# zuds-survey/zuds-pipeline

Measured on AMD Instinct MI355X. Metric: Mpix/s resample->coadd->subtract, 3072x3072 frames, higher is better.
Workload: dtype f32; 1 GPU; configs[1]+[2]: 32x 3072x3072 TPV frames/GPU, mesh background + weight rescale + Lanczos-3 resample + WEIGHTED coadd (+ AND mask coadd, int16 masks); then 1 science frame/GPU: align ref, hotpants 3x3 regions x 10x10 stamps, r=10, ko=4, subtract; frames_per_gpu=32, size=3072, mask_dtype=int16, combine=WEIGHTED, subtract=True

## Files before the change

### zuds-pipeline_amd/csrc/background.hip

```cpp
#include <algorithm>

#include "zm_internal.h"

#define BK_BIG 1e30f
#define BK_NLEVELS 4096
#define BK_THREADS 256

__device__ inline double block_sum(double v, double* red) {
#pragma unroll
    for (int o = 32; o >= 1; o >>= 1) v += __shfl_xor(v, o);
    const int wave = threadIdx.x >> 6;
    __syncthreads();
    if ((threadIdx.x & 63) == 0) red[wave] = v;
    __syncthreads();
    return (red[0] + red[1]) + (red[2] + red[3]);
}

#define BK_PER (BK_NLEVELS / BK_THREADS)

struct mesh_lds {
    int histo[BK_NLEVELS];
    long long b1[BK_THREADS];
    long long b2[BK_THREADS];
    double red[4];
// ... 200 lines not shown
    }
    __syncthreads();
    if ((threadIdx.x & 63) == 0) {
        red[0][threadIdx.x >> 6] = a;
        red[1][threadIdx.x >> 6] = b;
        red[2][threadIdx.x >> 6] = c;
    }
    __syncthreads();
    a = b = c = 0.0;
#pragma unroll
    for (int w = 0; w < BKF_WAVES; ++w) { a += red[0][w]; b += red[1][w]; c += red[2][w]; }
}

#define BK_BATCH 64
struct bk_batch {
    const float* img[BK_BATCH];
    const float* wgt[BK_BATCH];
};

__device__ __forceinline__ void mesh_general(float (&v)[BKF_PX], const int area, meshf_lds* S,
                                             mesh_dump* __restrict__ D, const int dbg, const float khint,
                                             const int rot0) {
    const int tid = threadIdx.x;
    const float qnan = __builtin_nanf("");
    float kf = khint;
    if (!(khint == khint)) {
#pragma unroll
    for (int k = BKF_PX - 1; k >= 0; --k) kf = (v[k] == v[k]) ? v[k] : kf;
    {
        const unsigned long long has = __ballot(kf == kf);
        const int src = has ? __ffsll((long long)has) - 1 : 0;
        kf = __shfl(kf, src);
        __syncthreads();
        if ((tid & 63) == 0) S->red[tid >> 6] = (double)kf;
        __syncthreads();
        double kd = __builtin_nan("");
#pragma unroll
        for (int w8 = BKF_WAVES - 1; w8 >= 0; --w8) { const double c = S->red[w8]; kd = (c == c) ? c : kd; }
        kf = (float)kd;
    }
    }
    if (!(kf == kf)) {
        if (tid == 0) D->valid = 0;
        return;
    }
    const double K = (double)kf;
    for (int k = tid; k < BK_NLEVELS; k += BKF_THREADS) S->histo[k] = 0;
    double s0 = 0, s1 = 0, s2 = 0;
    {
        int cnt = 0;
#pragma unroll
        for (int k = 0; k < BKF_PX; ++k) {
            const float x = v[k];
            const bool in = (x == x);
            const double d = (double)(in ? x : kf) - K;
            cnt += in ? 1 : 0;
            s1 += d;
            s2 = fma(d, d, s2);
        }
        s0 = (double)cnt;
    }
    blockf_sum3_1b(s0, s1, s2, S->rot[rot0 % 3]);
    if (s0 < area * 0.5 || s0 < 1.0) {
        if (tid == 0) D->valid = 0;
        return;
    }
    double dm = s1 / s0;
    double var = s2 / s0 - dm * dm;
    double sig = var > 0 ? sqrt(var) : 0.0;
    const bool allsame = sig == 0.0;
    const double lc = K + dm - 2.0 * sig, hc = K + dm + 2.0 * sig;
    s0 = s1 = s2 = 0;
    {
        float lcf = (float)lc, hcf = (float)hc;
        if ((double)lcf < lc) lcf = nextafterf(lcf, INFINITY);
        if ((double)hcf > hc) hcf = nextafterf(hcf, -INFINITY);
        int cnt = 0;
#pragma unroll
        for (int k = 0; k < BKF_PX; ++k) {
            const float x = v[k];
            const bool in = (x >= lcf) && (x <= hcf);
            const double d = (double)(in ? x : kf) - K;
            cnt += in ? 1 : 0;
            s1 += d;
            s2 = fma(d, d, s2);
        }
        s0 = (double)cnt;
    }
    blockf_sum3_1b(s0, s1, s2, S->rot[(rot0 + 1) % 3]);
    if (s0 < 1.0) {
        if (tid == 0) D->valid = 0;
        return;
    }
    dm = s1 / s0;
    const double mean = K + dm;
    var = s2 / s0 - dm * dm;
    sig = var > 0 ? sqrt(var) : 0.0;
    const bk_quant q = make_quant(mean, sig, s0);
    if (dbg == 2) { if (sig == 12345.0) D->valid = 7; return; }
    if (allsame) {
        if (tid == 0) {
                        D->q = q;
            D->mean0 = (double)(float)mean;
            D->valid = 2;
        }
        return;
    }
    {
        const float qinv = 1.0f / q.qscale;
        const bool slow_div = (__float_as_uint(q.qscale) & 0x7fffffu) == 0x7fffffu;
        if (!slow_div) {
#pragma unroll
            for (int k = 0; k < BKF_PX; ++k) {
                const float x = v[k];
                const float q0 = x * qinv;
                const float qq = fmaf(fmaf(-q0, q.qscale, x), qinv, q0);
                const int b = (int)(qq + q.cste);
                if ((x == x) && b >= 0 && b < q.nlevels) atomicAdd(&S->histo[b], 1);
            }
        } else {
#pragma unroll
            for (int k = 0; k < BKF_PX; ++k) {
                const float x = v[k];
                const int b = (int)(x / q.qscale + q.cste);
                if ((x == x) && b >= 0 && b < q.nlevels) atomicAdd(&S->histo[b], 1);
            }
        }
    }
    __syncthreads();
    if (dbg == 3) { if (S->histo[tid] == -5) D->valid = 7; return; }
    {
        constexpr int NB = BK_NLEVELS / BKF_THREADS;
        static_assert(NB == 8 || NB == 4, "the histogram hand-over packs 8 or 4 bins per thread");
        const int4 lo = *reinterpret_cast<const int4*>(&S->histo[NB * tid]);
        if (NB == 8) {
            const int4 hi = *reinterpret_cast<const int4*>(&S->histo[NB * tid + 4]);
            int4 o;
            o.x = (int)((unsigned)lo.x | ((unsigned)lo.y << 16));
            o.y = (int)((unsigned)lo.z | ((unsigned)lo.w << 16));
            o.z = (int)((unsigned)hi.x | ((unsigned)hi.y << 16));
            o.w = (int)((unsigned)hi.z | ((unsigned)hi.w << 16));
            reinterpret_cast<int4*>(D->h)[tid] = o;
        } else {
            int2 o;
            o.x = (int)((unsigned)lo.x | ((unsigned)lo.y << 16));
            o.y = (int)((unsigned)lo.z | ((unsigned)lo.w << 16));
            reinterpret_cast<int2*>(D->h)[tid] = o;
        }
        if (tid == 0) { D->q = q; D->mean0 = (double)(float)mean; D->valid = 1; }
    }
}

#ifndef BKF_WPS
#define BKF_WPS 4
#endif
template <int SEL>
__global__ __launch_bounds__(BKF_THREADS, BKF_WPS) void k_mesh_stats_fast(const bk_batch B, int nx, int ny, int mesh,
                                                                 int nbx, int nby, float wthresh, int vec_ok,
                                                                 int dbg, mesh_dump* __restrict__ dump) {
    extern __shared__ char smem_raw[];
    meshf_lds* S = reinterpret_cast<meshf_lds*>(smem_raw);
    constexpr int NM = SEL == 2 ? 2 : 1;
    const int frame = blockIdx.z;
    const float* __restrict__ img = B.img[frame];
    const float* __restrict__ wgt = B.wgt[frame];
    const int mi = blockIdx.x, mj = blockIdx.y;
    const int x0 = mi * mesh, y0 = mj * mesh;
    const int w = min(mesh, nx - x0), h = min(mesh, ny - y0);
    const int area = w * h;
    const int tid = threadIdx.x;
    const float qnan = __builtin_nanf("");
    mesh_dump* D0 = dump + ((size_t)(frame * NM) * nby + mj) * nbx + mi;
    mesh_dump* D1 = D0 + (size_t)(NM - 1) * nby * nbx;

    float v[BKF_PX];
    float wmn = __builtin_inff(), wmx = -__builtin_inff();
    int wcnt = 0;
    const float pinf = __builtin_inff();
    const float thr = wgt ? wthresh : -pinf;
    float khint = qnan;
    if (SEL != 1) {
        const size_t i00 = (size_t)y0 * nx + x0;
        const float p0 = img[i00], w0 = wgt ? wgt[i00] : 1.f;
        khint = (w0 > thr && fabsf(p0) < BK_BIG) ? p0 : qnan;
    }
    const int c4 = (tid & 31) * 4, r32 = tid >> 5;
#pragma unroll
    for (int k = 0; k < BKF_PX / 4; ++k) {
        const int row = BKF_ROWS * k + r32;
        float pv[4] = {qnan, qnan, qnan, qnan};
        float pw[4] = {-pinf, -pinf, -pinf, -pinf};
        if (row < h && c4 < w) {
            const size_t idx = (size_t)(y0 + row) * nx + x0 + c4;
            if (vec_ok && c4 + 3 < w) {
                if (SEL != 1) {
                    float4 a = *reinterpret_cast<const float4*>(img + idx);
                    pv[0] = a.x; pv[1] = a.y; pv[2] = a.z; pv[3] = a.w;
                }
                if (wgt) {
                    float4 b = *reinterpret_cast<const float4*>(wgt + idx);
                    pw[0] = b.x; pw[1] = b.y; pw[2] = b.z; pw[3] = b.w;
                } else {
                    pw[0] = pw[1] = pw[2] = pw[3] = 1.f;
                }
            } else {
#pragma unroll
                for (int j = 0; j < 4; ++j)
                    if (c4 + j < w) {
                        if (SEL != 1) pv[j] = img[idx + j];
                        pw[j] = wgt ? wgt[idx + j] : 1.f;
                    }
            }
        }
#pragma unroll
        for (int j = 0; j < 4; ++j) {
            const float x = pw[j];
            const bool good = x > thr;
            if (SEL != 0) {
                const bool in = good && (x > -BK_BIG);
                wmn = fminf(wmn, in ? x : pinf);
                wmx = fmaxf(wmx, in ? x : -pinf);
                wcnt += in ? 1 : 0;
                if (SEL == 1) v[4 * k + j] = in ? x : qnan;
            }
            if (SEL != 1) {
                const float val = pv[j];
                v[4 * k + j] = (good && (fabsf(val) < BK_BIG)) ? val : qnan;
            }
        }
    }
    if (dbg == 1) {
        float a = 0.f;
#pragma unroll
        for (int k = 0; k < BKF_PX; ++k) a += v[k];
        if (a == 12345.f) dump[0].valid = 7;
        return;
    }
    bool flat = false;
    if (SEL != 0) {
#pragma unroll
        for (int o = 32; o >= 1; o >>= 1) {
            wmn = fminf(wmn, __shfl_xor(wmn, o));
            wmx = fmaxf(wmx, __shfl_xor(wmx, o));
            wcnt += __shfl_xor(wcnt, o);
        }
        if ((tid & 63) == 0) { S->red3[0][tid >> 6] = wmn; S->red3[1][tid >> 6] = wmx; S->red3[2][tid >> 6] = wcnt; }
        __syncthreads();
        double bmn = S->red3[0][0], bmx = S->red3[1][0], bc = 0.0;
#pragma unroll
        for (int w8 = 0; w8 < BKF_WAVES; ++w8) {
            bmn = fmin(bmn, S->red3[0][w8]);
            bmx = fmax(bmx, S->red3[1][w8]);
            bc += S->red3[2][w8];
        }
        const float inv = 1.0f / (float)bmn;
        flat = bc >= 1.0 && bc >= area * 0.5 && bmn == bmx && inv > -BK_BIG && inv == inv;
        if (flat && tid == 0) {
            D1->q = make_quant((double)inv, 0.0, bc);
            D1->mean0 = (double)inv;
            D1->valid = 2;
        }
    }
    if (SEL != 1) mesh_general(v, area, S, D0, dbg, khint, 0);
    if (SEL == 0 || flat) return;
    if (SEL == 2) {
        __syncthreads();
#pragma unroll
        for (int k = 0; k < BKF_PX / 4; ++k) {
            const int row = BKF_ROWS * k + r32;
#pragma unroll
            for (int j = 0; j < 4; ++j) {
                float x = qnan;
                if (row < h && c4 + j < w) x = wgt[(size_t)(y0 + row) * nx + x0 + c4 + j];
                v[4 * k + j] = (x > wthresh && x > -BK_BIG) ? x : qnan;
            }
        }
    }
#pragma unroll
    for (int k = 0; k < BKF_PX; ++k) {
        const float x = v[k];
        const float val = 1.0f / x;
        const bool ok = (x == x) && (fabsf(val) < BK_BIG);
        v[k] = ok ? val : qnan;
    }
    __syncthreads();
    mesh_general(v, area, S, D1, dbg, qnan, 2);
}

__global__ __launch_bounds__(64) void k_mesh_guess(const mesh_dump* __restrict__ dump, int n, int nmode,
                                                   int nslot, float* __restrict__ raw) {
    __shared__ __attribute__((aligned(16))) unsigned short P0[BK_NLEVELS];
    __shared__ long long B1[BK_THREADS];
    __shared__ long long B2[BK_THREADS];
    const int m = blockIdx.x, z = blockIdx.y, lane = threadIdx.x;
    const int frame = z / nmode, mode = z - frame * nmode;
    const mesh_dump* D = dump + (size_t)z * n + m;
    float* ob = raw + (size_t)frame * 4 * nslot + (size_t)mode * 2 * n + m;
    float* os = ob + n;
    if (!D->valid) {
        if (lane == 0) { *ob = -BK_BIG; *os = -BK_BIG; }
        return;
    }
    if (D->valid == 2) {
        if (lane == 0) { *ob = D->q.qzero; *os = 0.f; }
        return;
    }
    const int4* src = reinterpret_cast<const int4*>(D->h);
    int4 piece[BK_NLEVELS / 8 / 64];
#pragma unroll
    for (int k = 0; k < BK_NLEVELS / 8 / 64; ++k) piece[k] = src[k * 64 + lane];
    unsigned run0 = 0;
    long long run1 = 0, run2 = 0;
#pragma unroll
    for (int k = 0; k < BK_NLEVELS / 8 / 64; ++k) {
        const unsigned wv[4] = {(unsigned)piece[k].x, (unsigned)piece[k].y, (unsigned)piece[k].z, (unsigned)piece[k].w};
        unsigned c[8];
#pragma unroll
        for (int j = 0; j < 4; ++j) { c[2 * j] = wv[j] & 0xffffu; c[2 * j + 1] = wv[j] >> 16; }
        unsigned s0 = 0, s1 = 0, s2 = 0;
#pragma unroll
        for (int j = 0; j < 8; ++j) { s0 += c[j]; s1 += c[j] * (unsigned)j; s2 += c[j] * (unsigned)(j * j); }
        const long long base = (long long)(512 * k + 8 * lane);
        const long long a1 = base * s0 + s1, a2 = base * base * s0 + 2 * base * s1 + s2;
        unsigned e0 = s0;
        long long e1 = a1, e2 = a2;
#pragma unroll
        for (int o = 1; o < 64; o <<= 1) {
            const unsigned t0 = __shfl_up(e0, o);
            const long long t1 = __shfl_up(e1, o), t2 = __shfl_up(e2, o);
            if (lane >= o) { e0 += t0; e1 += t1; e2 += t2; }
        }
        unsigned p = run0 + e0 - s0;
        unsigned w16[4];
#pragma unroll
        for (int j = 0; j < 4; ++j) {
            p += c[2 * j];
            const unsigned lo16 = p;
            p += c[2 * j + 1];
            w16[j] = lo16 | (p << 16);
        }
        reinterpret_cast<int4*>(P0)[k * 64 + lane] = make_int4((int)w16[0], (int)w16[1], (int)w16[2], (int)w16[3]);
        if ((lane & 1) == 0) {
            B1[32 * k + (lane >> 1)] = run1 + e1 - a1;
            B2[32 * k + (lane >> 1)] = run2 + e2 - a2;
        }
        run0 += __shfl(e0, 63);
        run1 += __shfl(e1, 63);
        run2 += __shfl(e2, 63);
    }
    __syncthreads();
    backguess_wave(P0, B1, B2, D->q, D->mean0, ob, os);
}

__global__ __launch_bounds__(BK_THREADS) void k_mesh_stats(const float* __restrict__ img,
                                                           const float* __restrict__ wgt,
                                                           int nx, int ny, int mesh, int nbx,
                                                           int nby, float wthresh, int mode0,
                                                           float* __restrict__ raw) {
    extern __shared__ char smem_raw[];
    mesh_lds* S = reinterpret_cast<mesh_lds*>(smem_raw);
    const int mode = mode0 + blockIdx.z;
    const int mi = blockIdx.x, mj = blockIdx.y;
    const int x0 = mi * mesh, y0 = mj * mesh;
    const int w = min(mesh, nx - x0), h = min(mesh, ny - y0);
    const int area = w * h;
    const int tid = threadIdx.x;
    float* ob = raw + (size_t)blockIdx.z * 2 * nbx * nby + (size_t)mj * nbx + mi;
    float* os = ob + (size_t)nbx * nby;

    auto value = [&](int k, bool* ok) -> float {
        int yy = k / w, xx = k - yy * w;
        size_t idx = (size_t)(y0 + yy) * nx + (x0 + xx);
        float v;
        bool good = true;
        if (mode == 0) {
            v = img[idx];
            if (wgt) good = wgt[idx] > wthresh;
        } else {
            float ww = wgt[idx];
            good = ww > wthresh;
            v = good ? 1.0f / ww : 0.f;
        }
        good = good && (fabsf(v) < BK_BIG);
        *ok = good;
        return v;
    };

    double s0 = 0, s1 = 0, s2 = 0;
    for (int k = tid; k < area; k += BK_THREADS) {
        bool ok;
        float v = value(k, &ok);
        if (ok) { s0 += 1.0; s1 += v; }
    }
    s0 = block_sum(s0, S->red);
    s1 = block_sum(s1, S->red);
    if (s0 < area * 0.5 || s0 < 1.0) {
        if (tid == 0) { *ob = -BK_BIG; *os = -BK_BIG; }
        return;
    }
    double mean = s1 / s0;
    for (int k = tid; k < area; k += BK_THREADS) {
        bool ok;
        float v = value(k, &ok);
        if (ok) { double dlt = (double)v - mean; s2 += dlt * dlt; }
    }
    s2 = block_sum(s2, S->red);
    double var = s2 / s0;
    double sig = var > 0 ? sqrt(var) : 0.0;
    const double lc = mean - 2.0 * sig, hc = mean + 2.0 * sig;
    s0 = s1 = s2 = 0;
    for (int k = tid; k < area; k += BK_THREADS) {
        bool ok;
        float v = value(k, &ok);
        if (ok && v >= lc && v <= hc) { s0 += 1.0; s1 += v; }
    }
    s0 = block_sum(s0, S->red);
    s1 = block_sum(s1, S->red);
    if (s0 < 1.0) {
        if (tid == 0) { *ob = -BK_BIG; *os = -BK_BIG; }
        return;
    }
    mean = s1 / s0;
    for (int k = tid; k < area; k += BK_THREADS) {
        bool ok;
        float v = value(k, &ok);
        if (ok && v >= lc && v <= hc) { double dlt = (double)v - mean; s2 += dlt * dlt; }
    }
    s2 = block_sum(s2, S->red);
    var = s2 / s0;
    sig = var > 0 ? sqrt(var) : 0.0;
    const bk_quant q = make_quant(mean, sig, s0);
    for (int k = tid; k < BK_NLEVELS; k += BK_THREADS) S->histo[k] = 0;
    __syncthreads();
    for (int k = tid; k < area; k += BK_THREADS) {
        bool ok;
        float v = value(k, &ok);
        if (ok) {
            int b = (int)(v / q.qscale + q.cste);
            if (b >= 0 && b < q.nlevels) atomicAdd(&S->histo[b], 1);
// ... 190 lines not shown
        for (int e = tid; e < 4 * nby; e += 1024) {
            const int m = e / (2 * nby), r = e - m * 2 * nby;
            const int which = r / nby, row = r - which * nby;
            float* P = pl + m * 4 * n;
            spline_line(P + which * n + row * nbx, P + (2 + which) * n + row * nbx,
                        tmp + (2 * m + which) * n + row * nbx, nbx, 1);
        }
        __syncthreads();
        for (int k = tid; k < 8 * n; k += 1024) nodes[k] = pl[k];
        return;
    }
    for (int m = 0; m < 2; ++m) {
        const float* fb = m ? fb1 : fb0;
        for (int k = tid; k < n; k += 1024) {
            float v = fb[k];
            int less = 0, eq = 0;
            for (int q = 0; q < n; ++q) { float o = fb[q]; less += o < v; eq += o == v; }
            int i1 = (n - 1) / 2, i2 = n / 2;
            if (i1 >= less && i1 < less + eq) med[2 * m] = v;
            if (i2 >= less && i2 < less + eq) med[2 * m + 1] = v;
        }
    }
    __syncthreads();
    if (tid == 0) {
        stats[0] = 0.5f * (med[0] + med[1]);
        stats[1] = 0.5f * (med[2] + med[3]);
    }
    for (int m = 0; m < 2; ++m) {
        const float* fb = m ? fb1 : fb0;
        float* V = pl;
        float* DY = pl + n;
        float* A = pl + 2 * n;
        float* B = pl + 3 * n;
        __syncthreads();
        for (int k = tid; k < n; k += 1024) V[k] = fb[k];
        __syncthreads();
        for (int i = tid; i < nbx; i += 1024) spline_line(V + i, DY + i, tmp + i, nby, nbx);
        __syncthreads();
        for (int j = tid; j < nby; j += 1024) spline_line(V + j * nbx, A + j * nbx, tmp + j * nbx, nbx, 1);
        __syncthreads();
        for (int j = tid; j < nby; j += 1024) spline_line(DY + j * nbx, B + j * nbx, tmp + j * nbx, nbx, 1);
        __syncthreads();
        float* out = nodes + (size_t)m * 4 * n;
        for (int k = tid; k < 4 * n; k += 1024) out[k] = pl[k];
    }
}

__device__ inline float bk_eval2(const float* __restrict__ bk, int nbx, int nby, float invmesh,
                                 int x, int y) {
    size_t pl = (size_t)nbx * nby;
    float ty = (y + 0.5f) * invmesh - 0.5f;
    float tx = (x + 0.5f) * invmesh - 0.5f;
    int j0 = 0, i0 = 0;
    float dy = 0.f, dx = 0.f;
    if (nby > 1) { j0 = min(max((int)floorf(ty), 0), nby - 2); dy = ty - j0; }
    if (nbx > 1) { i0 = min(max((int)floorf(tx), 0), nbx - 2); dx = tx - i0; }
    int j1 = nby > 1 ? j0 + 1 : j0, i1 = nbx > 1 ? i0 + 1 : i0;
    float dy1 = 1.f - dy, dx1 = 1.f - dx;
    float cdy = dy * dy * dy - dy, cdy1 = dy1 * dy1 * dy1 - dy1;
    float cdx = dx * dx * dx - dx, cdx1 = dx1 * dx1 * dx1 - dx1;
    const float* V = bk; const float* DY = bk + pl; const float* A = bk + 2 * pl; const float* B = bk + 3 * pl;
    int a00 = j0 * nbx + i0, a01 = j0 * nbx + i1, a10 = j1 * nbx + i0, a11 = j1 * nbx + i1;
    float r0 = dy1 * V[a00] + dy * V[a10] + cdy1 * DY[a00] + cdy * DY[a10];
    float r1 = dy1 * V[a01] + dy * V[a11] + cdy1 * DY[a01] + cdy * DY[a11];
    float e0 = dy1 * A[a00] + dy * A[a10] + cdy1 * B[a00] + cdy * B[a10];
    float e1 = dy1 * A[a01] + dy * A[a11] + cdy1 * B[a01] + cdy * B[a11];
    return dx1 * r0 + dx * r1 + cdx1 * e0 + cdx * e1;
}

__global__ __launch_bounds__(256) void k_bk_expand(const float* __restrict__ img,
                                                   const float* __restrict__ nodes, int nx,
                                                   int ny, int nbx, int nby, float invmesh,
                                                   float* __restrict__ out_bkg,
                                                   float* __restrict__ out_rms,
                                                   float* __restrict__ out_sub) {
    int x = blockIdx.x * blockDim.x + threadIdx.x, y = blockIdx.y;
    if (x >= nx) return;
    size_t idx = (size_t)y * nx + x;
    float b = bk_eval2(nodes, nbx, nby, invmesh, x, y);
    if (out_bkg) out_bkg[idx] = b;
    if (out_sub) out_sub[idx] = img[idx] - b;
    if (out_rms) out_rms[idx] = bk_eval2(nodes + (size_t)4 * nbx * nby, nbx, nby, invmesh, x, y);
}

__global__ void k_var_scale(const float* __restrict__ bstats, const float* __restrict__ vstats,
                            float* __restrict__ out) {
    float backsig = bstats[1], level = vstats[0];
    out[0] = (level > 0.f && backsig > 0.f) ? backsig * backsig / level : 1.f;
}

__global__ void k_var_scale_batch(const float* __restrict__ stats, float* __restrict__ out, int nf) {
    const int f = blockIdx.x * blockDim.x + threadIdx.x;
    if (f >= nf) return;
    const float backsig = stats[4 * f + 1], level = stats[4 * f + 2];
    out[4 * f] = (level > 0.f && backsig > 0.f) ? backsig * backsig / level : 1.f;
}

static int frame_slots(zm_ctx* ctx, int nx, int ny, int mesh, const char* slot, int index, int count,
                       int nslot, int* nbx_out, int* nby_out, float** raw, float** nodes, float** stats) {
    const int nbx = (nx - 1) / mesh + 1, nby = (ny - 1) / mesh + 1;
    const int n = nbx * nby;
    ZM_CHECK(n <= BK_MAXMESH, "background: %d x %d meshes exceed %d; raise BACK_SIZE", nbx, nby,
             BK_MAXMESH);
    if (nslot < n) nslot = n;
    std::string s(slot);
    ZM_TRY(ctx->get((s + "_raw").c_str(), sizeof(float) * 2 * 2 * nslot * (size_t)count, (void**)raw));
    ZM_TRY(ctx->get((s + "_nodes").c_str(), sizeof(float) * 2 * 8 * nslot * (size_t)count, (void**)nodes));
    ZM_TRY(ctx->get((s + "_stats").c_str(), sizeof(float) * 4 * (size_t)count, (void**)stats));
    *raw += (size_t)index * 2 * 2 * nslot;
    *nodes += (size_t)index * 2 * 8 * nslot;
    *stats += (size_t)index * 4;
    *nbx_out = nbx;
    *nby_out = nby;
    return 0;
}

int zm_batch_stats(zm_ctx* ctx, int nf, const float* const* imgs, const float* const* wgts, int nx,
                   int ny, int mesh, float wthresh, int mode0, int nmode, const char* slot, int index0,
                   int count, int nslot) {
    ZM_CHECK(mesh >= 8 && mesh <= 4096, "background: BACK_SIZE %d out of range [8, 4096]", mesh);
    ZM_CHECK(nmode >= 1 && mode0 >= 0 && mode0 + nmode <= 2, "background: bad statistic selection");
    ZM_CHECK(nf >= 1 && index0 >= 0 && index0 + nf <= count, "background: bad frame range");
    for (int f = 0; f < nf; ++f) {
        ZM_CHECK(mode0 + nmode < 2 || wgts[f] != nullptr, "background: the variance level needs a weight map");
        ZM_CHECK(mode0 > 0 || imgs[f] != nullptr, "background: image is NULL");
    }
    int nbx, nby;
    float *raw = nullptr, *nodes = nullptr, *stats = nullptr;
    ZM_TRY(frame_slots(ctx, nx, ny, mesh, slot, index0, count, nslot, &nbx, &nby, &raw, &nodes, &stats));
    const int n = nbx * nby;
    if (nslot < n) nslot = n;
    if (!ctx->bk_stats_set) {
        ZM_HIP(hipFuncSetAttribute((const void*)k_mesh_stats, hipFuncAttributeMaxDynamicSharedMemorySize,
                                   (int)sizeof(mesh_lds)));
        ctx->bk_stats_set = true;
    }
    zm_scope_timer t(ctx, "mesh_stats");
    if (mesh <= 128) {
        static const int dbg = ZM_DEVENV("ZM_DBG_BK") ? atoi(ZM_DEVENV("ZM_DBG_BK")) : 0;
        for (int f0 = 0; f0 < nf; f0 += BK_BATCH) {
            const int nb = std::min(BK_BATCH, nf - f0);
            bk_batch B;
            memset(&B, 0, sizeof(B));
            int vec_ok = (mesh % 4 == 0) && (nx % 4 == 0);
            for (int f = 0; f < nb; ++f) {
                B.img[f] = imgs[f0 + f];
                B.wgt[f] = wgts[f0 + f];
                if (((uintptr_t)B.img[f] & 15) || ((uintptr_t)B.wgt[f] & 15)) vec_ok = 0;
            }
            mesh_dump* dump = nullptr;
            ZM_TRY(ctx->get((std::string(slot) + "_dump").c_str(),
                            sizeof(mesh_dump) * 2 * (size_t)n * std::min(nf, BK_BATCH), (void**)&dump));
            const dim3 grid(nbx, nby, nb), block(BKF_THREADS, 1, 1);
            if (nmode == 2)
                hipLaunchKernelGGL(k_mesh_stats_fast<2>, grid, block, sizeof(meshf_lds), ctx->stream, B, nx, ny, mesh,
                                   nbx, nby, wthresh, vec_ok, dbg, dump);
            else if (mode0 == 0)
                hipLaunchKernelGGL(k_mesh_stats_fast<0>, grid, block, sizeof(meshf_lds), ctx->stream, B, nx, ny, mesh,
                                   nbx, nby, wthresh, vec_ok, dbg, dump);
            else
                hipLaunchKernelGGL(k_mesh_stats_fast<1>, grid, block, sizeof(meshf_lds), ctx->stream, B, nx, ny, mesh,
                                   nbx, nby, wthresh, vec_ok, dbg, dump);
            if (!ctx->bk_stats_event) ZM_HIP(hipEventCreateWithFlags(&ctx->bk_stats_event, hipEventDisableTiming));
            ZM_HIP(hipEventRecord(ctx->bk_stats_event, ctx->stream));
            ctx->bk_stats_event_valid = true;
            hipLaunchKernelGGL(k_mesh_guess, dim3(n, nmode * nb, 1), dim3(64, 1, 1), 0, ctx->stream,
                               dump, n, nmode, nslot, raw + (size_t)f0 * 4 * nslot);
        }
    } else {
        for (int f = 0; f < nf; ++f)
            hipLaunchKernelGGL(k_mesh_stats, dim3(nbx, nby, nmode), dim3(BK_THREADS, 1, 1),
                               sizeof(mesh_lds), ctx->stream, imgs[f], wgts[f], nx, ny, mesh, nbx, nby,
                               wthresh, mode0, raw + (size_t)f * 4 * nslot);
    }
    ZM_HIP(hipGetLastError());
    return 0;
}

int zm_batch_filter(zm_ctx* ctx, int nf, int nx, int ny, int mesh, int fsize, int nmode,
                    const char* slot, int index0, int count, int nslot) {
    ZM_CHECK(fsize >= 1 && fsize <= 7, "background: BACK_FILTERSIZE %d out of range [1, 7]", fsize);
    int nbx, nby;
    float *raw = nullptr, *nodes = nullptr, *stats = nullptr;
    ZM_TRY(frame_slots(ctx, nx, ny, mesh, slot, index0, count, nslot, &nbx, &nby, &raw, &nodes, &stats));
    const int n = nbx * nby;
    if (nslot < n) nslot = n;
    const bool fast = n <= 1024;
    const size_t fsh = sizeof(float) * (fast ? (size_t)8 * n + std::max(8 * n, 2048) : (size_t)9 * n);
    if (!ctx->bk_filter_set) {
        ZM_HIP(hipFuncSetAttribute((const void*)k_mesh_filter<false>,
                                   hipFuncAttributeMaxDynamicSharedMemorySize, 160 * 1024 - 64));
        ZM_HIP(hipFuncSetAttribute((const void*)k_mesh_filter<true>,
                                   hipFuncAttributeMaxDynamicSharedMemorySize, 160 * 1024 - 64));
        ctx->bk_filter_set = true;
    }
    zm_scope_timer t(ctx, "mesh_filter");
    if (fast)
        hipLaunchKernelGGL(k_mesh_filter<true>, dim3(nmode * nf, 1, 1), dim3(1024, 1, 1), fsh, ctx->stream,
                           raw, nbx, nby, fsize, nmode, nslot, nodes, stats);
    else
        hipLaunchKernelGGL(k_mesh_filter<false>, dim3(nmode * nf, 1, 1), dim3(1024, 1, 1), fsh, ctx->stream,
                           raw, nbx, nby, fsize, nmode, nslot, nodes, stats);
    ZM_HIP(hipGetLastError());
    return 0;
}

int zm_frame_products(zm_ctx* ctx, int nx, int ny, int mesh, const char* slot, int index, int count,
                      int nslot, float** nodes_dev, float** stats_dev, int* nbx_out, int* nby_out) {
    float* raw = nullptr;
    return frame_slots(ctx, nx, ny, mesh, slot, index, count, nslot, nbx_out, nby_out, &raw, nodes_dev,
                       stats_dev);
}

int zm_batch_var_scale(zm_ctx* ctx, int nf, const float* stats, float* out) {
    hipLaunchKernelGGL(k_var_scale_batch, dim3(zm_div_up(nf, 64)), dim3(64), 0, ctx->stream, stats, out, nf);
    ZM_HIP(hipGetLastError());
    return 0;
}

int zm_frame_stats(zm_ctx* ctx, const float* img, const float* wgt, int nx, int ny, int mesh,
                   float wthresh, int mode0, int nmode, const char* slot, int index, int count) {
    return zm_batch_stats(ctx, 1, &img, &wgt, nx, ny, mesh, wthresh, mode0, nmode, slot, index, count, 0);
}

int zm_frame_filter(zm_ctx* ctx, int nx, int ny, int mesh, int fsize, int nmode, float** nodes_dev,
                    float** stats_dev, int* nbx_out, int* nby_out, const char* slot, int index,
                    int count) {
    ZM_TRY(zm_batch_filter(ctx, 1, nx, ny, mesh, fsize, nmode, slot, index, count, 0));
    return zm_frame_products(ctx, nx, ny, mesh, slot, index, count, 0, nodes_dev, stats_dev, nbx_out, nby_out);
}

int zm_frame_background(zm_ctx* ctx, const float* img, const float* wgt, int nx, int ny,
                        int mesh, int fsize, float wthresh, int mode0, int nmode,
                        float** nodes_dev, float** stats_dev, int* nbx_out, int* nby_out,
                        const char* slot, int index, int count) {
    ZM_CHECK(fsize >= 1 && fsize <= 7, "background: BACK_FILTERSIZE %d out of range [1, 7]", fsize);
    ZM_TRY(zm_frame_stats(ctx, img, wgt, nx, ny, mesh, wthresh, mode0, nmode, slot, index, count));
    return zm_frame_filter(ctx, nx, ny, mesh, fsize, nmode, nodes_dev, stats_dev, nbx_out, nby_out,
                           slot, index, count);
}

int zm_launch_var_scale(zm_ctx* ctx, const float* bstats, const float* vstats, float* out) {
    hipLaunchKernelGGL(k_var_scale, dim3(1), dim3(1), 0, ctx->stream, bstats, vstats, out);
    ZM_HIP(hipGetLastError());
    return 0;
}

extern "C" int zm_background_dev(zm_ctx* ctx, const float* img, const float* wgt, int nx, int ny,
                                 int mesh, int filtersize, float* out_bkg, float* out_rms,
                                 float* out_sub, double* out_stats_host) {
    ZM_CHECK(ctx && img, "zm_background_dev: null argument");
    ZM_CHECK(nx > 0 && ny > 0, "zm_background_dev: empty image");
    ZM_HIP(hipSetDevice(ctx->device));
    float *nodes = nullptr, *stats = nullptr;
    int nbx = 0, nby = 0;
    ZM_TRY(zm_frame_background(ctx, img, wgt, nx, ny, mesh, filtersize, 1e-30f, 0, 1, &nodes, &stats,
                               &nbx, &nby, "bkg"));
    if (out_bkg || out_rms || out_sub) {
        zm_scope_timer t(ctx, "bk_expand");
        hipLaunchKernelGGL(k_bk_expand, dim3(zm_div_up(nx, 256), ny, 1), dim3(256, 1, 1), 0,
                           ctx->stream, img, nodes, nx, ny, nbx, nby, 1.0f / mesh, out_bkg,
                           out_rms, out_sub);
        ZM_HIP(hipGetLastError());
    }
    if (out_stats_host) {
        float hs[2];
        ZM_HIP(hipMemcpyAsync(hs, stats, sizeof(hs), hipMemcpyDeviceToHost, ctx->stream));
        ZM_HIP(hipStreamSynchronize(ctx->stream));
        out_stats_host[0] = hs[0];
        out_stats_host[1] = hs[1];
    }
    return 0;
}

extern "C" int zm_background(zm_ctx* ctx, const float* img, const float* wgt, int nx, int ny,
                             int mesh, int filtersize, float* out_bkg, float* out_rms,
                             float* out_sub, double* out_stats) {
    ZM_CHECK(ctx && img, "zm_background: null argument");
    ZM_CHECK(nx > 0 && ny > 0, "zm_background: empty image");
    ZM_HIP(hipSetDevice(ctx->device));
    const size_t np = (size_t)nx * ny;
    float *d_img = nullptr, *d_wgt = nullptr, *d_b = nullptr, *d_r = nullptr, *d_s = nullptr;
    ZM_TRY(ctx->get("h_img", np * 4, (void**)&d_img));
    ZM_HIP(hipMemcpyAsync(d_img, img, np * 4, hipMemcpyHostToDevice, ctx->stream));
    if (wgt) {
        ZM_TRY(ctx->get("h_wgt", np * 4, (void**)&d_wgt));
        ZM_HIP(hipMemcpyAsync(d_wgt, wgt, np * 4, hipMemcpyHostToDevice, ctx->stream));
    }
    if (out_bkg) ZM_TRY(ctx->get("h_oimg", np * 4, (void**)&d_b));
    if (out_rms) ZM_TRY(ctx->get("h_owgt", np * 4, (void**)&d_r));
    if (out_sub) ZM_TRY(ctx->get("h_osub", np * 4, (void**)&d_s));
    ZM_TRY(zm_background_dev(ctx, d_img, d_wgt, nx, ny, mesh, filtersize, d_b, d_r, d_s, out_stats));
    if (out_bkg) ZM_HIP(hipMemcpyAsync(out_bkg, d_b, np * 4, hipMemcpyDeviceToHost, ctx->stream));
    if (out_rms) ZM_HIP(hipMemcpyAsync(out_rms, d_r, np * 4, hipMemcpyDeviceToHost, ctx->stream));
    if (out_sub) ZM_HIP(hipMemcpyAsync(out_sub, d_s, np * 4, hipMemcpyDeviceToHost, ctx->stream));
    ZM_HIP(hipStreamSynchronize(ctx->stream));
    return 0;
}
```

### zuds-pipeline_amd/csrc/zm_internal.h

```cpp
#pragma once
#include <hip/hip_runtime.h>
#include <cstdint>
#include <cstdio>
#include <cstring>
#include <map>
#include <string>
#include <vector>
#include <stdexcept>

#include "../../include/zudsmi.h"

#define ZM_BIGVAR 1e30f
#define ZM_BADVAR_TEST 1e14f
#define ZM_SNAP 1e-5f

void zm_set_error(const char* fmt, ...);

#ifdef ZM_DEV
#define ZM_DEVENV(name) getenv(name)
#define ZM_DEV_BUILD 1
#else
#define ZM_DEVENV(name) ((const char*)nullptr)
#define ZM_DEV_BUILD 0
#endif

#define ZM_HIP(call)                                                         \
    do {                                                                     \
        hipError_t e_ = (call);                                              \
        if (e_ != hipSuccess) {                                              \
            zm_set_error("%s failed: %s (%s:%d)", #call, hipGetErrorString(e_), \
                         __FILE__, __LINE__);                                \
            return 1;                                                        \
        }                                                                    \
    } while (0)

#define ZM_CHECK(cond, ...)                                                  \
    do {                                                                     \
        if (!(cond)) {                                                       \
            zm_set_error(__VA_ARGS__);                                       \
            return 2;                                                        \
        }                                                                    \
    } while (0)

#define ZM_TRY(expr)                                                         \
    do {                                                                     \
        int r_ = (expr);                                                     \
        if (r_) return r_;                                                   \
    } while (0)

struct zm_timer_slot {
    double total_ms = 0.0;
    int64_t launches = 0;
    std::vector<std::pair<hipEvent_t, hipEvent_t>> pending;
};

struct zm_ctx {
    int device = 0;
    hipStream_t stream = nullptr;
    bool own_stream = true;
    std::map<std::string, std::pair<void*, size_t>> scratch;
    std::map<std::string, std::pair<void*, size_t>> pinned;
    hipStream_t aux = nullptr;
    std::vector<hipEvent_t> sync_events;
    const void* box_ready_for = nullptr;
    int box_ready_nt = 0;
    int share = 1;
    int hp_wg_cap = 0;
    bool hp_rset = false, hp_bset = false;
    hipEvent_t hp_done = nullptr;
    unsigned long long *hp_sig_h = nullptr, *hp_sig_d = nullptr;
    unsigned hp_seq = 0;
    bool hp_pending = false;
    int hp_pend_rounds = 0, hp_pend_retries = 0, hp_pend_nreg = 0, hp_pend_nunk = 0;
    std::map<int, size_t> hp_set_max;
    std::vector<double> hp_filt_host;
    const void* hp_filt_dev = nullptr;
    bool ff_pre_valid = false;
    int ff_pre_nfr = 0, ff_pre_onx = 0, ff_pre_ony = 0, ff_pre_lds = 0;
    bool ff_pre_own = false;
    int edge = 0;
    int mask_resample = 0;
    int ff_last_form = 0;
    bool bk_stats_set = false, bk_filter_set = false;
    hipEvent_t bk_stats_event = nullptr;
    bool bk_stats_event_valid = false;
    int cl_npre = 0;
    hipEvent_t lc_tab_event = nullptr;
    bool timing = false;
    std::string timing_only;
    std::map<std::string, zm_timer_slot> timers;
    std::vector<hipEvent_t> event_pool;

    int get(const char* name, size_t bytes, void** out);
    int get_pinned(const char* name, size_t bytes, void** out);
    void release_all();
};

struct zm_scope_timer {
    zm_ctx* ctx;
    const char* name;
    hipEvent_t a = nullptr, b = nullptr;
    zm_scope_timer(zm_ctx* c, const char* n);
    ~zm_scope_timer();
};

static inline int zm_div_up(int a, int b) { return (a + b - 1) / b; }

#define ZM_LATTICE_STEP 16

struct zm_map_params {
    zm_wcs wout;
    zm_wcs win;
    double rot[9];
};

void zm_wcs_frame(const zm_wcs* w, double fr[9]);
void zm_make_map(const zm_wcs* wout, const zm_wcs* win, zm_map_params* mp);
void zm_map_point(const zm_map_params* mp, double xo, double yo, double* xi, double* yi);
double zm_pixel_area(const zm_wcs* w, double x, double y);
void zm_wcs_pix2vec(const zm_wcs* w, const double* fr, double x, double y, double v[3]);
void zm_wcs_mark_order(zm_wcs* w);

int zm_launch_lattice(zm_ctx* ctx, const zm_map_params* mp, int lnx, int lny, double2* lat_dev);
int zm_launch_lattice_batch(zm_ctx* ctx, const zm_map_params* mp_host, int n, int lnx, int lny,
                            double2* lat_dev, hipEvent_t after = nullptr);
int zm_launch_prep(zm_ctx* ctx, const float* img, const float* wgt, int nx, int ny,
                   const float* bknodes, int nbx, int nby, int mesh,
                   const float* var_scale_dev, float wthresh, float2* dst, int spitch,
                   const int32_t* mask_for_box = nullptr, int box_nt = 0, uint16_t* mbox_out = nullptr,
                   int mbox_pitch = 0);
struct zm_ff {
    const float* img;
    const float* wgt;
    const float4* ytab;
    const float4* xtab;
    const float* vscale;
    const float2* src;
    const double2* lat;
    const void* mask;
    const uint16_t* mbox;
    const float* bk;
    const int* mboxflag;
    int nx, ny, spitch, nbx, nby, ytp;
    float invmesh, wthresh, fscale, fscale2;
    int vec_ok, mpitch;
    int mask16, pad_;
};
struct zm_bkrows {
    const float* bk;
    float4* out;
    int nbx, nby, ny, ytp;
    float invmesh;
    int nx;
    float4* xout;
};
struct zm_boxjob {
    const void* m;
    uint16_t* B;
    int* rawflag;
    int nx, ny, pitch, is16;
};
void zm_fused_geometry(int* tile_h, int* lds_cap);
int zm_launch_fused_prepass(zm_ctx* ctx, const zm_bkrows* rows, int nrows);
int zm_launch_mask_boxes(zm_ctx* ctx, const zm_boxjob* boxes, int nboxes, hipEvent_t after, hipEvent_t* joined,
                         hipEvent_t after2 = nullptr);
int zm_launch_fused_headers_early(zm_ctx* ctx, const zm_ff* frames_host, int nfr, int lnx, int lny, int onx, int ony,
                                  int lds_elems, bool fits_own);
int zm_launch_coadd_fused(zm_ctx* ctx, const zm_ff* frames_host, int nfr, int lnx, int lny, int onx, int ony,
                          int lds_elems, int combine, int mask_kind, float* out_img, float* out_wgt,
                          int32_t* out_mask, float* out_cov, int partial, int32_t* unmasked_out,
                          float2* stack = nullptr, int64_t fstride = 0, bool fits_own = false);
int zm_get_lanczos_table(zm_ctx* ctx, const float** out);
int zm_check_wcs(const zm_wcs* w, const char* what);
int zm_resample_lds_plan(const zm_map_params* mp, int onx, int ony, int kernel);
int zm_frame_background(zm_ctx* ctx, const float* img, const float* wgt, int nx, int ny,
                        int mesh, int fsize, float wthresh, int mode0, int nmode,
                        float** nodes_dev, float** stats_dev, int* nbx_out, int* nby_out,
                        const char* slot, int index = 0, int count = 1);
int zm_batch_stats(zm_ctx* ctx, int nf, const float* const* imgs, const float* const* wgts, int nx,
                   int ny, int mesh, float wthresh, int mode0, int nmode, const char* slot, int index0,
                   int count, int nslot);
int zm_batch_filter(zm_ctx* ctx, int nf, int nx, int ny, int mesh, int fsize, int nmode,
                    const char* slot, int index0, int count, int nslot);
int zm_frame_products(zm_ctx* ctx, int nx, int ny, int mesh, const char* slot, int index, int count,
                      int nslot, float** nodes_dev, float** stats_dev, int* nbx_out, int* nby_out);
int zm_batch_var_scale(zm_ctx* ctx, int nf, const float* stats, float* out);
int zm_frame_stats(zm_ctx* ctx, const float* img, const float* wgt, int nx, int ny, int mesh,
                   float wthresh, int mode0, int nmode, const char* slot, int index, int count);
int zm_frame_filter(zm_ctx* ctx, int nx, int ny, int mesh, int fsize, int nmode, float** nodes_dev,
                    float** stats_dev, int* nbx_out, int* nby_out, const char* slot, int index,
                    int count);
int zm_get_sync_events(zm_ctx* ctx, int n, hipEvent_t** out);
hipStream_t zm_ctx_aux(zm_ctx* ctx);
int zm_launch_var_scale(zm_ctx* ctx, const float* bstats, const float* vstats, float* out);
int zm_launch_resample(zm_ctx* ctx, const float2* src, int nx, int ny, int spitch,
                       const double2* lat, int lnx, int lny, int kernel, float fscale,
                       float2* dst, int onx, int ony, int lds_elems, const int32_t* mask,
                       int32_t* macc, int mop, int mkind, int mfirst,
                       float* plane_a = nullptr, float* plane_b = nullptr, float pair_scale = 0.f);
int zm_launch_prep_pair(zm_ctx* ctx, const float* a, const float* b, int nx, int ny, float2* dst, int spitch);
int zm_launch_resample_mask(zm_ctx* ctx, const int32_t* mask, int nx, int ny,
                            const double2* lat, int lnx, int lny, int kernel,
                            int32_t* dst, int onx, int ony, int32_t fill);
int zm_launch_combine(zm_ctx* ctx, int n, const float2* stack, int64_t frame_stride,
                      int64_t npix, int kind, float clip_sigma, float clip_ampfrac,
                      float* out_img, float* out_wgt, int partial);
int zm_launch_resample_rim(zm_ctx* ctx, const float2* src, int nx, int ny, int spitch, const double2* lat, int lnx,
                           int lny, int kernel, float fscale, float2* dst, float* plane_a, float* plane_b, int onx,
                           int ony, const int32_t* mask, int32_t* macc, int mop, int mkind);
int zm_launch_resample_mask_opts(zm_ctx* ctx, const int32_t* mask, int nx, int ny, const double2* lat, int lnx, int lny,
                                 int kernel, int32_t* dst, int onx, int ony, int32_t fill, int lanczos, int trunc);
int zm_launch_mask_accum(zm_ctx* ctx, int32_t* acc, const int32_t* m, int64_t npix, int kind,
                         int first);
int zm_launch_mask_finalize(zm_ctx* ctx, int32_t* acc, float* cov, int64_t npix);
int zm_launch_split_pairs(zm_ctx* ctx, const float2* src, int64_t npix, float* a, float* b);
int zm_launch_mask_widen(zm_ctx* ctx, const int16_t* in, int64_t n, int32_t* out);

#define EX_OI 8
struct zm_ex_bufs {
    float* filt;
    int *seg, *label, *cnt, *bad32;
    int* small;
    int np, nsb;
};
int zm_ex_check(zm_ctx* ctx, const float* img, const float* sigma, int nx, int ny, const zm_extract_params* params,
                int max_objects, const zm_object* out_rows, const int* out_nwritten, const int* out_nfound);
int zm_ex_planes(zm_ctx* ctx, int nx, int ny, int32_t* segm_dev, float* filtered_dev, zm_ex_bufs* b);
void zm_ex_label(zm_ctx* ctx, const float* img, const float* sigma, const uint8_t* bad, int nx, int ny,
                 const zm_extract_params* params, const zm_ex_bufs* b);
int zm_ex_recount(zm_ctx* ctx, const int* label, const zm_ex_bufs* b);
void zm_ex_count_roots(zm_ctx* ctx, const int* label, int minarea, const zm_ex_bufs* b);
void zm_ex_number(zm_ctx* ctx, const int* label, const float* img, const int32_t* flag, int nx, int ny,
                  const zm_extract_params* params, int cap, int* seg, int* obj, const zm_ex_bufs* b);
int zm_ex_rows(zm_ctx* ctx, const float* img, const float* sigma, int nx, int ny, const zm_wcs* wcs,
               const zm_extract_params* params, int n, const int* d_seg, const int* d_obj, const zm_ex_bufs* b,
               zm_object* out_rows);
// ... 11 lines not shown
```

Before: 49470 Mpix/s.

## Defer non-flat weight-variance mesh stats to a compacted persistent kernel

The two-mode mesh statistics kernel now handles only the image statistics and the flat-weight fast path. Non-flat weight meshes are appended to a device-side work list through an atomic counter. A second persistent kernel then processes that list with a grid-stride loop and a double-buffered counter. This lets the common kernel drop the weight reload and variance histogram, so it can run with higher occupancy (launch bound raised to 6 waves per SIMD). The cost is an extra kernel launch, atomics, and a second pass over the weights for the deferred meshes.

```diff
diff --git a/zuds-pipeline_amd/csrc/background.hip b/zuds-pipeline_amd/csrc/background.hip
--- a/zuds-pipeline_amd/csrc/background.hip
+++ b/zuds-pipeline_amd/csrc/background.hip
@@ -376,26 +376,23 @@
 }
 
 #ifndef BKF_WPS
-#define BKF_WPS 4
+#define BKF_WPS 6
 #endif
+#define BKF_WPS_VAR 4
+#define BKD_HDR 4
 template <int SEL>
-__global__ __launch_bounds__(BKF_THREADS, BKF_WPS) void k_mesh_stats_fast(const bk_batch B, int nx, int ny, int mesh,
-                                                                 int nbx, int nby, float wthresh, int vec_ok,
-                                                                 int dbg, mesh_dump* __restrict__ dump) {
-    extern __shared__ char smem_raw[];
-    meshf_lds* S = reinterpret_cast<meshf_lds*>(smem_raw);
-    constexpr int NM = SEL == 2 ? 2 : 1;
-    const int frame = blockIdx.z;
+__device__ __forceinline__ void mesh_stats_body(const bk_batch& B, meshf_lds* S, const int frame, const int mi,
+                                                const int mj, int nx, int ny, int mesh, int nbx, int nby,
+                                                float wthresh, int vec_ok, int dbg,
+                                                mesh_dump* __restrict__ dump, mesh_dump* __restrict__ D0,
+                                                mesh_dump* __restrict__ D1, int* __restrict__ defer, int turn) {
     const float* __restrict__ img = B.img[frame];
     const float* __restrict__ wgt = B.wgt[frame];
-    const int mi = blockIdx.x, mj = blockIdx.y;
     const int x0 = mi * mesh, y0 = mj * mesh;
     const int w = min(mesh, nx - x0), h = min(mesh, ny - y0);
     const int area = w * h;
     const int tid = threadIdx.x;
     const float qnan = __builtin_nanf("");
-    mesh_dump* D0 = dump + ((size_t)(frame * NM) * nby + mj) * nbx + mi;
-    mesh_dump* D1 = D0 + (size_t)(NM - 1) * nby * nbx;
 
     float v[BKF_PX];
     float wmn = __builtin_inff(), wmx = -__builtin_inff();
@@ -484,22 +481,13 @@
             D1->mean0 = (double)inv;
             D1->valid = 2;
         }
+        if (SEL == 2 && !flat && tid == 0) {
+            D1->valid = 0;
+            defer[BKD_HDR + atomicAdd(&defer[turn], 1)] = (frame * nby + mj) * nbx + mi;
+        }
     }
     if (SEL != 1) mesh_general(v, area, S, D0, dbg, khint, 0);
-    if (SEL == 0 || flat) return;
-    if (SEL == 2) {
-        __syncthreads();
-#pragma unroll
-        for (int k = 0; k < BKF_PX / 4; ++k) {
-            const int row = BKF_ROWS * k + r32;
-#pragma unroll
-            for (int j = 0; j < 4; ++j) {
-                float x = qnan;
-                if (row < h && c4 + j < w) x = wgt[(size_t)(y0 + row) * nx + x0 + c4 + j];
-                v[4 * k + j] = (x > wthresh && x > -BK_BIG) ? x : qnan;
-            }
-        }
-    }
+    if (SEL != 1 || flat) return;
 #pragma unroll
     for (int k = 0; k < BKF_PX; ++k) {
         const float x = v[k];
@@ -509,6 +497,36 @@
     }
     __syncthreads();
     mesh_general(v, area, S, D1, dbg, qnan, 2);
+}
+
+template <int SEL>
+__global__ __launch_bounds__(BKF_THREADS, SEL == 1 ? BKF_WPS_VAR : BKF_WPS) void k_mesh_stats_fast(
+    const bk_batch B, int nx, int ny, int mesh, int nbx, int nby, float wthresh, int vec_ok, int dbg,
+    mesh_dump* __restrict__ dump, int* __restrict__ defer, int turn) {
+    extern __shared__ char smem_raw[];
+    meshf_lds* S = reinterpret_cast<meshf_lds*>(smem_raw);
+    constexpr int NM = SEL == 2 ? 2 : 1;
+    const int frame = blockIdx.z, mi = blockIdx.x, mj = blockIdx.y;
+    mesh_dump* D0 = dump + ((size_t)(frame * NM) * nby + mj) * nbx + mi;
+    mesh_dump* D1 = D0 + (size_t)(NM - 1) * nby * nbx;
+    mesh_stats_body<SEL>(B, S, frame, mi, mj, nx, ny, mesh, nbx, nby, wthresh, vec_ok, dbg, dump, D0, D1, defer, turn);
+}
+
+__global__ __launch_bounds__(BKF_THREADS, BKF_WPS_VAR) void k_mesh_stats_deferred(
+    const bk_batch B, int nx, int ny, int mesh, int nbx, int nby, float wthresh, int vec_ok,
+    mesh_dump* __restrict__ dump, int* __restrict__ defer, int turn) {
+    extern __shared__ char smem_raw[];
+    meshf_lds* S = reinterpret_cast<meshf_lds*>(smem_raw);
+    const int count = defer[turn];
+    if (blockIdx.x == 0 && threadIdx.x == 0) defer[turn ^ 1] = 0;
+    for (int i = blockIdx.x; i < count; i += gridDim.x) {
+        const int e = defer[BKD_HDR + i];
+        const int mi = e % nbx, fj = e / nbx;
+        const int mj = fj % nby, frame = fj / nby;
+        mesh_dump* D1 = dump + ((size_t)(frame * 2 + 1) * nby + mj) * nbx + mi;
+        mesh_stats_body<1>(B, S, frame, mi, mj, nx, ny, mesh, nbx, nby, wthresh, vec_ok, 0, dump, D1, D1, nullptr, 0);
+        __syncthreads();
+    }
 }
 
 __global__ __launch_bounds__(64) void k_mesh_guess(const mesh_dump* __restrict__ dump, int n, int nmode,
@@ -1005,15 +1023,29 @@
             ZM_TRY(ctx->get((std::string(slot) + "_dump").c_str(),
                             sizeof(mesh_dump) * 2 * (size_t)n * std::min(nf, BK_BATCH), (void**)&dump));
             const dim3 grid(nbx, nby, nb), block(BKF_THREADS, 1, 1);
-            if (nmode == 2)
+            if (nmode == 2) {
+                const std::string dname = std::string(slot) + "_defer";
+                const auto had = ctx->scratch.find(dname);
+                const void* before = had != ctx->scratch.end() ? had->second.first : nullptr;
+                int* defer = nullptr;
+                ZM_TRY(ctx->get(dname.c_str(), sizeof(int) * (BKD_HDR + (size_t)n * std::min(nf, BK_BATCH)),
+                                (void**)&defer));
+                if ((const void*)defer != before) ZM_HIP(hipMemsetAsync(defer, 0, sizeof(int) * BKD_HDR, ctx->stream));
+                const int turn = (int)(ctx->bk_defer_turn[dname]++ & 1u);
                 hipLaunchKernelGGL(k_mesh_stats_fast<2>, grid, block, sizeof(meshf_lds), ctx->stream, B, nx, ny, mesh,
-                                   nbx, nby, wthresh, vec_ok, dbg, dump);
-            else if (mode0 == 0)
+                                   nbx, nby, wthresh, vec_ok, dbg, dump, defer, turn);
+                static int ncu[64] = {0};
+                int& cus = ncu[ctx->device & 63];
+                if (!cus) ZM_HIP(hipDeviceGetAttribute(&cus, hipDeviceAttributeMultiprocessorCount, ctx->device));
+                const int nwg = std::max(1, std::min(2 * cus, n * nb));
+                hipLaunchKernelGGL(k_mesh_stats_deferred, dim3(nwg, 1, 1), block, sizeof(meshf_lds), ctx->stream, B, nx,
+                                   ny, mesh, nbx, nby, wthresh, vec_ok, dump, defer, turn);
+            } else if (mode0 == 0)
                 hipLaunchKernelGGL(k_mesh_stats_fast<0>, grid, block, sizeof(meshf_lds), ctx->stream, B, nx, ny, mesh,
-                                   nbx, nby, wthresh, vec_ok, dbg, dump);
+                                   nbx, nby, wthresh, vec_ok, dbg, dump, (int*)nullptr, 0);
             else
                 hipLaunchKernelGGL(k_mesh_stats_fast<1>, grid, block, sizeof(meshf_lds), ctx->stream, B, nx, ny, mesh,
-                                   nbx, nby, wthresh, vec_ok, dbg, dump);
+                                   nbx, nby, wthresh, vec_ok, dbg, dump, (int*)nullptr, 0);
             if (!ctx->bk_stats_event) ZM_HIP(hipEventCreateWithFlags(&ctx->bk_stats_event, hipEventDisableTiming));
             ZM_HIP(hipEventRecord(ctx->bk_stats_event, ctx->stream));
             ctx->bk_stats_event_valid = true;
diff --git a/zuds-pipeline_amd/csrc/zm_internal.h b/zuds-pipeline_amd/csrc/zm_internal.h
--- a/zuds-pipeline_amd/csrc/zm_internal.h
+++ b/zuds-pipeline_amd/csrc/zm_internal.h
@@ -82,6 +82,7 @@
     int mask_resample = 0;
     int ff_last_form = 0;
     bool bk_stats_set = false, bk_filter_set = false;
+    std::map<std::string, unsigned> bk_defer_turn;
     hipEvent_t bk_stats_event = nullptr;
     bool bk_stats_event_valid = false;
     int cl_npre = 0;
```

After: 49750 Mpix/s (median of 6 runs). Within noise of the previous version (+0.6%).
